# pythoncrazy/jimm

Hardware: NVIDIA H100
Metric: images/sec (higher is better)
Workload: dtype f16

## Files before the change

### include/jimm_b200.h

```cpp
#ifndef JIMM_B200_H_
#define JIMM_B200_H_

#include <stddef.h>
#include <stdint.h>

#if defined(__GNUC__)
#define JIMM_API __attribute__((visibility("default")))
#else
#define JIMM_API
#endif

#ifdef __cplusplus
extern "C" {
#endif

typedef struct jimm_model jimm_model_t;

enum jimm_status { JIMM_OK = 0, JIMM_EINVAL = -1, JIMM_ECUDA = -2, JIMM_EDRIVER = -3, JIMM_ESTATE = -4, JIMM_ENOMEM = -5 };
enum jimm_dtype { JIMM_F32 = 0, JIMM_F16 = 1, JIMM_BF16 = 2, JIMM_I32 = 3 };
enum jimm_kind {
  JIMM_VIT = 0, JIMM_CLIP = 1, JIMM_SIGLIP = 2, JIMM_TOWER = 3 ,
  JIMM_ENCODER = 4 ,
  JIMM_MAPHEAD = 5
};
// ... 70 lines not shown
JIMM_API int jimm_k_layernorm_ex(const float* x, int ldx, int group, int row_off, const int32_t* row_index, const float* scale, const float* bias,
                                 float eps, void* out, int out_type, int ldy, int rows, int D, int reverse, void* stream);
JIMM_API int jimm_k_attention_ex(const void* qkv, int io_type, void* out, int out_type, int B, int S, int H, int causal, int reverse,
                                 void* stream);
JIMM_API int jimm_k_map_attention(const float* q, const void* kv, int io_type, void* out, int out_type, int B, int S, int H, void* stream);
JIMM_API int jimm_k_attention_hd(const void* qkv, int io_type, void* out, int out_type, int B, int S, int H, int head_dim, int causal,
                                 int reverse, void* stream);
JIMM_API int jimm_k_map_attention_hd(const float* q, const void* kv, int io_type, void* out, int out_type, int B, int S, int H, int head_dim,
                                     void* stream);
JIMM_API int jimm_k_patchify(const void* img, int in_type, int B, int H, int W, int C, int P, void* out, int out_type, void* stream);
JIMM_API int jimm_k_patchify_ex(const void* img, int in_type, int B, int H, int W, int C, int P, void* out, int out_type, int rows_per_sample,
                                int ldk, void* stream);
JIMM_API int jimm_k_activation(const float* x, float* y, long long n, int act, void* stream);
JIMM_API int jimm_k_embed(const int32_t* ids, const float* table, const float* pos, float* x, int B, int T, int D, int vocab, void* stream);
JIMM_API int jimm_k_l2_normalize(const float* x, float* out, int ldo, int B, int E, void* stream);
JIMM_API int jimm_k_logits(const float* img, const float* txt, const float* logit_scale, const float* logit_bias, float* logits, int Bi, int Bt,
                  int E, int ldl, void* stream);
typedef struct jimm_preproc_config {
  int height, width;
  int shortest_edge;
  int crop_h, crop_w;
  int resample;
  double rescale_factor;
  float mean[3], std[3];
} jimm_preproc_config_t;
JIMM_API int jimm_preproc_create(const jimm_preproc_config_t* cfg, int device, jimm_preproc_t** out);
JIMM_API int jimm_preproc_output_size(const jimm_preproc_t* p, int H, int W, int* out_h, int* out_w);
JIMM_API int jimm_preproc_run(jimm_preproc_t* p, const uint8_t* img, int B, int H, int W, void* out, int out_dtype, void* stream);
JIMM_API int jimm_preproc_destroy(jimm_preproc_t* p);
JIMM_API int jimm_k_resample_coeffs(int in_size, int out_size, int resample, int* ksize, int* first, int* count, int* kk, int kk_capacity);
JIMM_API int jimm_postprocess(const float* logits, int rows, int cols, int ld, int mode, float* probs, int ldp, int32_t* order, int32_t* argmax,
                              void* stream);
JIMM_API int jimm_k_l2_probe(const void* buf, int rows, int mode, int cluster, int iters, float* ms, void* stream);
JIMM_API int jimm_profile_begin(jimm_model_t* m);
JIMM_API int jimm_profile_end(jimm_model_t* m, double* gemm_ms, double* gemm_flops, long long* gemm_launches);
JIMM_API long long jimm_launch_count(void);
JIMM_API long long jimm_graph_replay_count(void);

#ifdef __cplusplus
}
#endif
#endif
```

### jimm_b200/_lib.py

```python

from __future__ import annotations

import ctypes as C
import os

_HERE = os.path.dirname(os.path.abspath(__file__))
LIB_PATH = os.path.join(_HERE, "libjimm_b200.so")

F32, F16, BF16, I32 = 0, 1, 2, 3
PARAM_TRANSPOSED = 1
KIND_VIT, KIND_CLIP, KIND_SIGLIP, KIND_TOWER, KIND_ENCODER, KIND_MAPHEAD = 0, 1, 2, 3, 4, 5
POOL_CLS, POOL_MAP = 0, 1
ACT_GELU_TANH, ACT_QUICK_GELU = 0, 1
TPOOL_EOT_ARGMAX, TPOOL_LAST = 0, 1


class Config(C.Structure):

    _fields_ = [
        ("kind", C.c_int),
        ("img_size", C.c_int), ("patch", C.c_int), ("in_ch", C.c_int), ("v_width", C.c_int), ("v_layers", C.c_int),
        ("v_heads", C.c_int), ("v_mlp", C.c_int),
        ("pooling", C.c_int),
        ("pre_norm", C.c_int), ("patch_bias", C.c_int), ("v_act", C.c_int),
# ... 35 lines not shown
    "jimm_contrastive_logits": (_i, [_vp, _fp, _i, _fp, _i, _fp, _vp]),
    "jimm_dual_encode": (_i, [_vp, _vp, _i, _i, _ip, _i, _i, _fp, _fp, _vp]),
    "jimm_dual_forward": (_i, [_vp, _vp, _i, _i, _ip, _i, _i, _fp, _vp]),
    "jimm_encoder_forward": (_i, [_vp, _fp, _i, _i, _fp, _vp]),
    "jimm_map_head_forward": (_i, [_vp, _fp, _i, _i, _fp, _vp]),
    "jimm_vit_forward_host": (_i, [_vp, _vp, _i, _i, _fp, _vp]),
    "jimm_dual_forward_host": (_i, [_vp, _vp, _i, _i, _ip, _i, _i, _fp, _vp]),
    "jimm_vit_forward_host_u8": (_i, [_vp, _vp, _vp, _i, _i, _i, _fp, _vp]),
    "jimm_comm_init": (_i, [_vp, _i, _i, _i, C.c_char_p]),
    "jimm_comm_connect": (_i, [_vp, C.c_char_p]),
    "jimm_comm_contrastive_logits": (_i, [_vp, _fp, _fp, _i, _fp, _vp]),
    "jimm_comm_status": (_i, [_vp]),
    "jimm_comm_gathered": (_i, [_vp, C.POINTER(_vp), C.POINTER(_i)]),
    "jimm_profile_begin": (_i, [_vp]),
    "jimm_profile_end": (_i, [_vp, C.POINTER(C.c_double), C.POINTER(C.c_double), C.POINTER(C.c_longlong)]),
    "jimm_k_gemm": (_i, [_i, _i, _vp, _i, _vp, _i, _i, _i, _i, _fp, _i, _fp, _fp, _i, _vp, _i, _i, _i, _i, _i, _i, _vp]),
    "jimm_k_gemm_residual_ln": (_i, [_i, _vp, _i, _vp, _i, _i, _i, _i, _fp, _fp, _i, _fp, _fp, _f, _vp, _i, _i, _ip, _vp]),
    "jimm_k_gemm_ex": (_i, [_i, _i, _vp, _i, _vp, _i, _i, _i, _i, _fp, _i, _fp, _fp, _i, _vp, _i, _i, _i, _i, _i, _i,
                            _i, _i, _i, _i, _i, _fp, _fp, _f, _vp, _i, _i, _ip, _vp]),
    "jimm_k_layernorm": (_i, [_fp, _i, _i, _i, _ip, _fp, _fp, _f, _vp, _i, _i, _i, _i, _vp]),
    "jimm_k_attention": (_i, [_vp, _i, _vp, _i, _i, _i, _i, _i, _vp]),
    "jimm_k_layernorm_ex": (_i, [_fp, _i, _i, _i, _ip, _fp, _fp, _f, _vp, _i, _i, _i, _i, _i, _vp]),
    "jimm_k_attention_ex": (_i, [_vp, _i, _vp, _i, _i, _i, _i, _i, _i, _vp]),
    "jimm_k_map_attention": (_i, [_fp, _vp, _i, _vp, _i, _i, _i, _i, _vp]),
    "jimm_k_attention_hd": (_i, [_vp, _i, _vp, _i, _i, _i, _i, _i, _i, _i, _vp]),
    "jimm_k_map_attention_hd": (_i, [_fp, _vp, _i, _vp, _i, _i, _i, _i, _i, _vp]),
    "jimm_k_patchify": (_i, [_vp, _i, _i, _i, _i, _i, _i, _vp, _i, _vp]),
    "jimm_k_patchify_ex": (_i, [_vp, _i, _i, _i, _i, _i, _i, _vp, _i, _i, _i, _vp]),
    "jimm_k_activation": (_i, [_fp, _fp, C.c_longlong, _i, _vp]),
    "jimm_k_embed": (_i, [_ip, _fp, _fp, _fp, _i, _i, _i, _i, _vp]),
    "jimm_k_l2_normalize": (_i, [_fp, _fp, _i, _i, _i, _vp]),
    "jimm_k_logits": (_i, [_fp, _fp, _fp, _fp, _fp, _i, _i, _i, _i, _vp]),
    "jimm_k_l2_probe": (_i, [_vp, _i, _i, _i, _i, C.POINTER(C.c_float), _vp]),
    "jimm_postprocess": (_i, [_fp, _i, _i, _i, _i, _fp, _i, _ip, _ip, _vp]),
    "jimm_preproc_create": (_i, [C.POINTER(PreprocConfig), _i, C.POINTER(_vp)]),
    "jimm_preproc_output_size": (_i, [_vp, _i, _i, C.POINTER(_i), C.POINTER(_i)]),
    "jimm_preproc_run": (_i, [_vp, _vp, _i, _i, _i, _vp, _i, _vp]),
    "jimm_preproc_destroy": (_i, [_vp]),
    "jimm_k_resample_coeffs": (_i, [_i, _i, _i, C.POINTER(_i), _ip, _ip, _ip, _i]),
}

_lib = None


class JimmError(RuntimeError):
    pass


def load():
    global _lib
    if _lib is not None:
        return _lib
    if not os.path.exists(LIB_PATH):
        raise JimmError(f"{LIB_PATH} not found: build it with `python -m jimm_b200.build` (there is no CPU fallback)")
    lib = C.CDLL(LIB_PATH)
    for name, (res, args) in SIGNATURES.items():
        fn = getattr(lib, name)
        fn.restype = res
        fn.argtypes = args
    _lib = lib
    return lib


def last_error() -> str:
    return load().jimm_last_error().decode("utf-8", "replace")

# ... 9 lines not shown
```

### jimm_b200/csrc/common.cuh

```cuda
#pragma once

#include <cuda.h>
#include <cuda_bf16.h>
#include <cuda_fp16.h>
#include <cuda_runtime.h>
#include <stdint.h>

namespace jimm {

void set_last_error(const char* fmt, ...);

#define JIMM_CUDA_CHECK(expr)                                                                   \
  do {                                                                                          \
    cudaError_t _e = (expr);                                                                    \
    if (_e != cudaSuccess) {                                                                    \
      ::jimm::set_last_error("%s:%d: %s -> %s", __FILE__, __LINE__, #expr, cudaGetErrorString(_e)); \
      return -2;                                                                                \
    }                                                                                           \
  } while (0)

void note_launch();
#define JIMM_LAUNCH_CHECK()                  \
  do {                                       \
    JIMM_CUDA_CHECK(cudaGetLastError());     \
// ... 83 lines not shown
  asm volatile(
      "{\n\t.reg .pred P1;\n\t"
      "WAIT_LOOP:\n\t"
      "mbarrier.try_wait.parity.shared::cta.b64 P1, [%0], %1;\n\t"
      "@P1 bra DONE;\n\t"
      "bra WAIT_LOOP;\n\t"
      "DONE:\n\t}" ::"r"(smem_u32(bar)),
      "r"(parity)
      : "memory");
}

__device__ __forceinline__ bool mbar_test_wait(uint64_t* bar, uint32_t parity) {
  uint32_t ok;
  asm volatile(
      "{\n\t.reg .pred P1;\n\t"
      "mbarrier.test_wait.parity.shared::cta.b64 P1, [%1], %2;\n\t"
      "selp.u32 %0, 1, 0, P1;\n\t}"
      : "=r"(ok)
      : "r"(smem_u32(bar)), "r"(parity)
      : "memory");
  return ok != 0;
}

__device__ __forceinline__ void tma_prefetch_desc(const CUtensorMap* m) {
  asm volatile("prefetch.tensormap [%0];" ::"l"(reinterpret_cast<uint64_t>(m)) : "memory");
}
__device__ __forceinline__ void tma_load_2d(void* smem_dst, const CUtensorMap* m, uint64_t* bar, int c0, int c1) {
  asm volatile(
      "cp.async.bulk.tensor.2d.shared::cluster.global.mbarrier::complete_tx::bytes [%0], [%1, {%3, %4}], [%2];" ::"r"(
          smem_u32(smem_dst)),
      "l"(reinterpret_cast<uint64_t>(m)), "r"(smem_u32(bar)), "r"(c0), "r"(c1)
      : "memory");
}

__device__ __forceinline__ void tma_store_2d(const CUtensorMap* m, uint32_t smem_src, int c0, int c1) {
  asm volatile("cp.async.bulk.tensor.2d.global.shared::cta.bulk_group [%0, {%2, %3}], [%1];" ::"l"(reinterpret_cast<uint64_t>(m)),
               "r"(smem_src), "r"(c0), "r"(c1)
               : "memory");
}
__device__ __forceinline__ void tma_reduce_add_2d(const CUtensorMap* m, uint32_t smem_src, int c0, int c1) {
  asm volatile("cp.reduce.async.bulk.tensor.2d.global.shared::cta.add.tile.bulk_group [%0, {%2, %3}], [%1];" ::"l"(
                   reinterpret_cast<uint64_t>(m)),
               "r"(smem_src), "r"(c0), "r"(c1)
               : "memory");
}
__device__ __forceinline__ void tma_store_3d(const CUtensorMap* m, uint32_t smem_src, int c0, int c1, int c2) {
  asm volatile("cp.async.bulk.tensor.3d.global.shared::cta.bulk_group [%0, {%2, %3, %4}], [%1];" ::"l"(reinterpret_cast<uint64_t>(m)),
               "r"(smem_src), "r"(c0), "r"(c1), "r"(c2)
               : "memory");
}
__device__ __forceinline__ void tma_reduce_add_3d(const CUtensorMap* m, uint32_t smem_src, int c0, int c1, int c2) {
  asm volatile("cp.reduce.async.bulk.tensor.3d.global.shared::cta.add.tile.bulk_group [%0, {%2, %3, %4}], [%1];" ::"l"(
                   reinterpret_cast<uint64_t>(m)),
               "r"(smem_src), "r"(c0), "r"(c1), "r"(c2)
               : "memory");
}
__device__ __forceinline__ void tma_store_commit() { asm volatile("cp.async.bulk.commit_group;" ::: "memory"); }
__device__ __forceinline__ void tma_store_wait_read() { asm volatile("cp.async.bulk.wait_group.read 0;" ::: "memory"); }
__device__ __forceinline__ void tma_store_wait_read1() { asm volatile("cp.async.bulk.wait_group.read 1;" ::: "memory"); }
__device__ __forceinline__ void tma_store_wait_all() { asm volatile("cp.async.bulk.wait_group 0;" ::: "memory"); }

__device__ __forceinline__ uint32_t cluster_ctarank() {
  uint32_t r;
  asm volatile("mov.u32 %0, %%cluster_ctarank;" : "=r"(r));
  return r;
}
__device__ __forceinline__ void cluster_sync_all() {
  asm volatile("barrier.cluster.arrive.release.aligned;\n\tbarrier.cluster.wait.acquire.aligned;" ::: "memory");
}
__device__ __forceinline__ uint32_t mapa_shared(uint32_t local_smem_addr, uint32_t rank) {
  uint32_t r;
  asm volatile("mapa.shared::cluster.u32 %0, %1, %2;" : "=r"(r) : "r"(local_smem_addr), "r"(rank));
  return r;
}
__device__ __forceinline__ void mbar_arrive_cluster(uint32_t cluster_addr) {
  asm volatile("mbarrier.arrive.release.cluster.shared::cluster.b64 _, [%0];" ::"r"(cluster_addr) : "memory");
}
__device__ __forceinline__ uint64_t make_wgmma_desc_sw128(uint32_t smem_addr) {
  uint64_t d = 0;
  d |= static_cast<uint64_t>((smem_addr & 0x3FFFFu) >> 4);
  d |= static_cast<uint64_t>(1) << 16;
  d |= static_cast<uint64_t>(1024 >> 4) << 32;
  d |= static_cast<uint64_t>(1) << 62;
  return d;
}
template <int SW>
__device__ __forceinline__ uint64_t make_wgmma_desc(uint32_t smem_addr, uint32_t lbo) {
  static_assert(SW == 128 || SW == 64 || SW == 32, "swizzle width");
  constexpr uint64_t layout = SW == 128 ? 1 : SW == 64 ? 2 : 3;
  uint64_t d = 0;
  d |= static_cast<uint64_t>((smem_addr & 0x3FFFFu) >> 4);
  d |= static_cast<uint64_t>((lbo >> 4) & 0x3FFFu) << 16;
  d |= static_cast<uint64_t>(8 * SW >> 4) << 32;
  d |= layout << 62;
  return d;
}
__device__ __forceinline__ void wgmma_fence() { asm volatile("wgmma.fence.sync.aligned;" ::: "memory"); }
__device__ __forceinline__ void wgmma_commit() { asm volatile("wgmma.commit_group.sync.aligned;" ::: "memory"); }
template <int N>
__device__ __forceinline__ void wgmma_wait() { asm volatile("wgmma.wait_group.sync.aligned %0;" ::"n"(N) : "memory"); }
template <int R>
__device__ __forceinline__ void wgmma_fence_operands(float (&d)[R]) {
#pragma unroll
  for (int i = 0; i < R; ++i) asm volatile("" : "+f"(d[i])::"memory");
}

#define JIMM_WGMMA_D128                                                                                                                    \
  "{%0, %1, %2, %3, %4, %5, %6, %7, %8, %9, %10, %11, %12, %13, %14, %15, %16, %17, %18, %19, %20, %21, %22, %23, %24, %25, %26, %27, "     \
  "%28, %29, %30, %31, %32, %33, %34, %35, %36, %37, %38, %39, %40, %41, %42, %43, %44, %45, %46, %47, %48, %49, %50, %51, %52, %53, %54, " \
// ... 252 lines not shown
```

### jimm_b200/csrc/gemm.cu

```cuda
#include "gemm.cuh"

#include <stdarg.h>
#include <stdio.h>
#include <stdlib.h>
#include <string.h>

#include <type_traits>

#include "common.cuh"

namespace jimm {

static constexpr int BM = GEMM_TILE_M;
static constexpr int BN = GEMM_TILE_N;
static_assert(BM == 128 && BN == 256, "the warp roles and the wgmma shape below are written for 128 x 256 tiles");
static constexpr int STAGES = 4;
static constexpr int A_STAGE_BYTES = BM * 128;
static constexpr int B_STAGE_BYTES = BN * 128;
static constexpr int STAGE_BYTES = A_STAGE_BYTES + B_STAGE_BYTES;
static constexpr int EPI_WARPS = 8;
static constexpr int EPI_BOX_ROWS = 16;
static constexpr int EPI_BUF_BYTES = EPI_BOX_ROWS * 128;
static constexpr int EPI_BUFS = 2;
static constexpr int EPI_STAGE_BYTES = EPI_WARPS * EPI_BUFS * EPI_BUF_BYTES;
static constexpr int NUM_THREADS = 384;
static constexpr int KERNEL_REGS = 168;

enum OutKind : int { OUT_GENERIC = 0, OUT_H16 = 1, OUT_BF16 = 2, OUT_TF32 = 3, OUT_F32_ADD = 4, OUT_F32 = 5 };

struct EpiDev {
  const float* bias;
  const float* rowadd;
  const float* residual;
  void* out;
  int act, ldr, out_type, ldo, rows_in, rows_out, row_off, mode;
  int M, N;
  int reverse;
  int tok_pad, tok_off;
  const float* ln_scale;
  const float* ln_bias;
  void* ln_out;
  int* ln_cnt;
  int ln_out_type, ln_ldo;
  float ln_eps;
};

template <int ACT>
__device__ __forceinline__ float act_ct(float v) {
// ... 252 lines not shown
          if (epi.residual) v += epi.residual[static_cast<size_t>(out_row) * epi.ldr + col];
          store1(epi, out_row, col, v);
        }
      }
    }
  }
}

template <typename T, int OUT, int ACT>
__global__ void __launch_bounds__(NUM_THREADS, 1)
gemm_wgmma_kernel(const __grid_constant__ CUtensorMap map_a, const __grid_constant__ CUtensorMap map_b,
                  const __grid_constant__ CUtensorMap map_c, const EpiDev epi, int K) {
  constexpr int BK = 128 / sizeof(T);
  constexpr int UK = 32 / sizeof(T);
  constexpr bool FUSE_LN = OUT == OUT_F32_ADD && ACT == ACT_FUSE_LN;
  constexpr int EPI_ACT = ACT == ACT_FUSE_LN ? static_cast<int>(ACT_NONE) : ACT;
  constexpr int PRODUCER_REGS = FUSE_LN ? 152 : 40;
  constexpr int CONSUMER_REGS = FUSE_LN ? 176 : 232;
  static_assert(128 * PRODUCER_REGS + 256 * CONSUMER_REGS <= NUM_THREADS * KERNEL_REGS, "register split exceeds the CTA's allocation");

  extern __shared__ uint8_t smem_raw[];
  uint8_t* smem = reinterpret_cast<uint8_t*>((reinterpret_cast<uintptr_t>(smem_raw) + 1023) & ~static_cast<uintptr_t>(1023));
  uint8_t* smem_a = smem;
  uint8_t* smem_b = smem + STAGES * A_STAGE_BYTES;
  uint8_t* epi_stage = smem + STAGES * STAGE_BYTES;
  LnQueue* lnq = reinterpret_cast<LnQueue*>(epi_stage + EPI_STAGE_BYTES);
  uint64_t* full_bar = reinterpret_cast<uint64_t*>(lnq + 1);
  uint64_t* empty_bar = full_bar + STAGES;

  const int warp_idx = threadIdx.x >> 5;
  const int lane = threadIdx.x & 31;
  const int M = epi.M, N = epi.N;
  const int m_tiles = (M + BM - 1) / BM, n_tiles = (N + BN - 1) / BN;
  const int num_tiles = m_tiles * n_tiles;
  const int num_kb = (K + BK - 1) / BK;

  pdl_launch_dependents();
  if (warp_idx == 0 && lane == 0) {
    tma_prefetch_desc(&map_a);
    tma_prefetch_desc(&map_b);
    if constexpr (OUT != OUT_GENERIC) tma_prefetch_desc(&map_c);
    for (int s = 0; s < STAGES; ++s) {
      mbar_init(&full_bar[s], 1);
      mbar_init(&empty_bar[s], EPI_WARPS);
    }
    fence_barrier_init();
  }
  if constexpr (FUSE_LN) {
    if (warp_idx == 1) {
      for (int i = lane; i < LNQ; i += 32) lnq->slot[i] = -1;
      if (lane == 0) lnq->head = lnq->tail = lnq->done = 0;
    }
  }
  __syncthreads();
  pdl_wait();

  if (warp_idx < 4) {
    setmaxnreg<KERNEL_REGS, PRODUCER_REGS>();
    if (warp_idx == 0) {
      if (lane == 0) {
        int stage = 0;
        uint32_t phase = 0;
        for (int tile = blockIdx.x; tile < num_tiles; tile += gridDim.x) {
          const int tv = epi.reverse ? num_tiles - 1 - tile : tile;
          const int m_blk = tv / n_tiles, n_blk = tv - m_blk * n_tiles;
          for (int kb = 0; kb < num_kb; ++kb) {
            mbar_wait(&empty_bar[stage], phase ^ 1);
            mbar_arrive_expect_tx(&full_bar[stage], STAGE_BYTES);
            tma_load_2d(smem_a + stage * A_STAGE_BYTES, &map_a, &full_bar[stage], kb * BK, m_blk * BM);
            tma_load_2d(smem_b + stage * B_STAGE_BYTES, &map_b, &full_bar[stage], kb * BK, n_blk * BN);
            if (++stage == STAGES) { stage = 0; phase ^= 1; }
          }
        }
      }
    } else if constexpr (FUSE_LN) {
      ln_worker<T>(epi, lnq, lane);
    }
  } else {
    setmaxnreg<KERNEL_REGS, CONSUMER_REGS>();
    const int wg = (warp_idx - 4) >> 2;
    const int wq = warp_idx & 3;
    uint8_t* tbuf0 = epi_stage + (warp_idx - 4) * EPI_BUFS * EPI_BUF_BYTES;
    int stage = 0;
    uint32_t phase = 0, box_count = 0;
    int ln_rg = -1, ln_cols = 0;
    float acc[128];
    for (int tile = blockIdx.x; tile < num_tiles; tile += gridDim.x) {
      const int tv = epi.reverse ? num_tiles - 1 - tile : tile;
      const int m_blk = tv / n_tiles, n_blk = tv - m_blk * n_tiles;
      int prev = -1;
      for (int kb = 0; kb < num_kb; ++kb) {
        mbar_wait(&full_bar[stage], phase);
        const uint64_t adesc = make_wgmma_desc_sw128(smem_u32(smem_a + stage * A_STAGE_BYTES + wg * 64 * 128));
        const uint64_t bdesc = make_wgmma_desc_sw128(smem_u32(smem_b + stage * B_STAGE_BYTES));
        wgmma_fence_operands(acc);
        wgmma_fence();
#pragma unroll
        for (int k = 0; k < BK / UK; ++k)
          wgmma_m64n256_ss<Traits<T>::KIND>(acc, adesc + static_cast<uint64_t>(2 * k), bdesc + static_cast<uint64_t>(2 * k), (kb | k) != 0 ? 1u : 0u);
        wgmma_commit();
        wgmma_fence_operands(acc);
        if (prev >= 0) {
          wgmma_wait<1>();
          if (lane == 0) mbar_arrive(&empty_bar[prev]);
        }
        prev = stage;
        if (++stage == STAGES) { stage = 0; phase ^= 1; }
      }
      wgmma_wait<0>();
      wgmma_fence_operands(acc);
      if (lane == 0) mbar_arrive(&empty_bar[prev]);

      const int row_base = m_blk * BM + wg * 64 + wq * 16;
      const int n_tile0 = n_blk * BN;
      if constexpr (OUT == OUT_GENERIC) {
        epilogue_generic(epi, acc, lane, row_base, n_tile0);
      } else {
        if (row_base < M) epilogue_tma<OUT, EPI_ACT>(&map_c, epi, acc, tbuf0, lane, row_base, n_tile0, box_count);
        if constexpr (FUSE_LN) {
          if (lane == 0 && ln_rg >= 0) ln_publish(epi, lnq, ln_rg, ln_cols);
          ln_rg = (row_base & ~31) < M ? row_base >> 5 : -1;
          ln_cols = min(BN, N - n_tile0);
        }
      }
    }
    if constexpr (FUSE_LN) {
      if (lane == 0) {
        if (ln_rg >= 0) ln_publish(epi, lnq, ln_rg, ln_cols);
        __threadfence_block();
        atomicAdd(&lnq->done, 1);
      }
    }
    if constexpr (OUT != OUT_GENERIC) {
      if (lane == 0) tma_store_wait_all();
    }
  }
}

template <typename T>
__global__ void gemm_simt_kernel(const T* __restrict__ A, int lda, const T* __restrict__ B, int ldb, int K, EpiDev epi) {
  __shared__ float As[16][17], Bs[16][17];
  const int tx = threadIdx.x, ty = threadIdx.y;
  const int row = blockIdx.y * 16 + ty, col = blockIdx.x * 16 + tx;
  float acc = 0.f;
  for (int k0 = 0; k0 < K; k0 += 16) {
    const int ar = blockIdx.y * 16 + ty, ak = k0 + tx;
    As[ty][tx] = (ar < epi.M && ak < K) ? to_float(A[static_cast<size_t>(ar) * lda + ak]) : 0.f;
    const int br = blockIdx.x * 16 + ty, bk = k0 + tx;
    Bs[ty][tx] = (br < epi.N && bk < K) ? to_float(B[static_cast<size_t>(br) * ldb + bk]) : 0.f;
    __syncthreads();
#pragma unroll
    for (int k = 0; k < 16; ++k) acc += As[ty][k] * Bs[tx][k];
    __syncthreads();
  }
  if (row < epi.M && col < epi.N) {
    int out_row, add_row;
    remap_row(epi, row, out_row, add_row);
    float v = acc;
    if (epi.bias) v += epi.bias[col];
    v = apply_act(v, epi.act);
    if (epi.rowadd) v += epi.rowadd[static_cast<size_t>(add_row) * epi.N + col];
    if (epi.residual) v += epi.residual[static_cast<size_t>(out_row) * epi.ldr + col];
    store1(epi, out_row, col, v);
  }
}

static constexpr int SMEM_BYTES = STAGES * STAGE_BYTES + EPI_STAGE_BYTES + static_cast<int>(sizeof(LnQueue)) + 2 * STAGES * 8 + 1024;
static_assert(SMEM_BYTES <= 232448, "exceeds 227 KB of shared memory");
typedef CUresult (*PFN_encodeTiled)(CUtensorMap*, CUtensorMapDataType, cuuint32_t, void*, const cuuint64_t*, const cuuint64_t*,
// ... 43 lines not shown
  const size_t es = dtype_size(dtype);
  CUtensorMapDataType dt = (dtype == DT_F32 || dtype == DT_TF32) ? CU_TENSOR_MAP_DATA_TYPE_FLOAT32
                                           : (dtype == DT_F16 ? CU_TENSOR_MAP_DATA_TYPE_FLOAT16 : CU_TENSOR_MAP_DATA_TYPE_BFLOAT16);
  cuuint64_t dims[3] = {static_cast<cuuint64_t>(N), static_cast<cuuint64_t>(S), static_cast<cuuint64_t>(B)};
  cuuint64_t strides[2] = {static_cast<cuuint64_t>(ld) * es, static_cast<cuuint64_t>(S) * ld * es};
  cuuint32_t box[3] = {static_cast<cuuint32_t>(128 / es), EPI_BOX_ROWS, 1};
  cuuint32_t estr[3] = {1, 1, 1};
  CUresult r = enc(map, dt, 3, const_cast<void*>(ptr), dims, strides, box, estr, CU_TENSOR_MAP_INTERLEAVE_NONE,
                   CU_TENSOR_MAP_SWIZZLE_128B, CU_TENSOR_MAP_L2_PROMOTION_L2_256B, CU_TENSOR_MAP_FLOAT_OOB_FILL_NONE);
  if (r != CUDA_SUCCESS) { set_last_error("cuTensorMapEncodeTiled(3d) failed: CUresult %d", static_cast<int>(r)); return -3; }
  return 0;
}
static int make_map_3d_f32(CUtensorMap* map, const void* ptr, int B, int S, int N, int ld) { return make_tensor_map_3d(map, DT_F32, ptr, B, S, N, ld); }

int make_tensor_map_2d(CUtensorMap* map, int dtype, const void* ptr, int rows, int cols, int ld, int box_rows) {
  return make_map(map, dtype, ptr, rows, cols, ld, box_rows);
}

int device_sm_count() {
  static int sms[DeviceOnce::kMaxDevices] = {};
  int dev = 0;
  cudaGetDevice(&dev);
  if (dev < 0 || dev >= DeviceOnce::kMaxDevices) dev = 0;
  if (sms[dev] == 0) {
    int n = 0;
    cudaDeviceGetAttribute(&n, cudaDevAttrMultiProcessorCount, dev);
    const char* env = getenv("JIMM_NUM_SMS");
    if (env && atoi(env) > 0) n = atoi(env);
    sms[dev] = n;
  }
  return sms[dev];
}

static int check_epi(const GemmEpilogue& e, int N) {
  if (e.out == nullptr) { set_last_error("gemm: null output"); return -1; }
  if (e.ldo < N) { set_last_error("gemm: ldo (%d) < N (%d)", e.ldo, N); return -1; }
  return 0;
}
int gemm_plan_init(GemmPlan* plan, int dtype, const void* A, int lda, const void* B, int ldb, int M, int N, int K,
                   const GemmEpilogue& epi) {
  if (M <= 0 || N <= 0 || K <= 0) { set_last_error("gemm: bad shape %dx%dx%d", M, N, K); return -1; }
  if (int rc = check_epi(epi, N)) return rc;
  if (epi.tok_pad != 0) {
    if (epi.tok_pad < 0 || epi.tok_pad % EPI_BOX_ROWS != 0 || M % epi.tok_pad != 0 || epi.tok_off < 0 || epi.tok_S <= 0) {
      set_last_error("gemm: token scatter needs tok_pad a positive multiple of %d dividing M (tok_pad=%d M=%d tok_off=%d tok_S=%d)", EPI_BOX_ROWS,
                     epi.tok_pad, M, epi.tok_off, epi.tok_S);
      return -1;
    }
    if (epi.residual != epi.out || epi.ldr != epi.ldo || epi.out_type != DT_F32) {
      set_last_error("gemm: token scatter reduce-adds into an fp32 output that is also the residual");
      return -1;
    }
  }
  if (int rc = make_map(&plan->map_a, dtype, A, M, K, lda, BM)) return rc;
  if (int rc = make_map(&plan->map_b, dtype, B, N, K, ldb, BN)) return rc;
  plan->M = M; plan->N = N; plan->K = K; plan->dtype = dtype; plan->epi = epi;
  memset(&plan->map_c, 0, sizeof(plan->map_c));
  if (plan->epi.mode == 2) {
    const size_t es = dtype_size(epi.out_type);
    const bool ok = epi.rowadd == nullptr && epi.rows_in == 0 && (static_cast<size_t>(N) * es) % 16 == 0 &&
                    (epi.residual == nullptr || (epi.residual == epi.out && epi.ldr == epi.ldo && epi.out_type == DT_F32)) &&
                    (static_cast<size_t>(epi.ldo) * es) % 16 == 0 && (reinterpret_cast<uintptr_t>(epi.out) & 15) == 0 &&
                    (epi.bias == nullptr || ((reinterpret_cast<uintptr_t>(epi.bias) & 15) == 0 && N % 4 == 0)) &&
                    !(epi.residual && epi.act != ACT_NONE);
    if (ok && epi.tok_pad > 0) {
      if (int rc = make_map_3d_f32(&plan->map_c, epi.out, M / epi.tok_pad, epi.tok_S, N, epi.ldo)) return rc;
    } else if (ok) {
      if (int rc = make_map(&plan->map_c, epi.out_type, epi.out, M, N, epi.ldo, EPI_BOX_ROWS)) return rc;
    } else {
      plan->epi.mode = 0;
    }
  }
  if (epi.tok_pad > 0 && plan->epi.mode != 2) {
    set_last_error("gemm: the token scatter needs the TMA epilogue (mode 2, no activation, 16-byte aligned output / bias, N %% 4 == 0)");
    return -1;
  }
  return 0;
}

static EpiDev to_dev(const GemmEpilogue& e, int M, int N) {
  EpiDev d;
  d.bias = e.bias; d.rowadd = e.rowadd; d.residual = e.residual; d.out = e.out;
  d.act = e.act; d.ldr = e.ldr; d.out_type = e.out_type; d.ldo = e.ldo;
  d.rows_in = e.rows_in; d.rows_out = e.rows_out; d.row_off = e.row_off; d.mode = e.mode;
  d.M = M; d.N = N;
  d.tok_pad = e.tok_pad; d.tok_off = e.tok_off;
  d.reverse = e.reverse;
  d.ln_scale = e.ln_scale; d.ln_bias = e.ln_bias; d.ln_out = e.ln_out; d.ln_cnt = e.ln_cnt;
  d.ln_out_type = e.ln_out_type; d.ln_ldo = e.ln_ldo; d.ln_eps = e.ln_eps;
  return d;
}

template <typename T, int OUT, int ACT>
static int launch_one(const GemmPlan* p, int M, cudaStream_t stream) {
  static DeviceOnce attr_set;
  if (attr_set.first()) {
    JIMM_CUDA_CHECK(cudaFuncSetAttribute(gemm_wgmma_kernel<T, OUT, ACT>, cudaFuncAttributeMaxDynamicSharedMemorySize, SMEM_BYTES));
    cudaFuncAttributes fa;
    JIMM_CUDA_CHECK(cudaFuncGetAttributes(&fa, gemm_wgmma_kernel<T, OUT, ACT>));
    if (fa.numRegs != KERNEL_REGS) {
      set_last_error("gemm: kernel compiled with %d registers per thread, the warpgroup register split assumes %d", fa.numRegs, KERNEL_REGS);
      return -2;
    }
  }
  const int tiles = ((M + BM - 1) / BM) * ((p->N + BN - 1) / BN);
  const int grid = tiles < device_sm_count() ? tiles : device_sm_count();
  JIMM_CUDA_CHECK(launch_k(gemm_wgmma_kernel<T, OUT, ACT>, dim3(grid), dim3(NUM_THREADS), SMEM_BYTES, stream, 1, true, p->map_a, p->map_b,
                           p->map_c, to_dev(p->epi, M, p->N), p->K));
  note_launch();
  return 0;
}

template <typename T, int OUT>
static int launch_act(const GemmPlan* p, int M, cudaStream_t stream) {
  switch (p->epi.act) {
    case ACT_GELU_TANH: return launch_one<T, OUT, ACT_GELU_TANH>(p, M, stream);
    case ACT_QUICK_GELU: return launch_one<T, OUT, ACT_QUICK_GELU>(p, M, stream);
    default: return launch_one<T, OUT, ACT_NONE>(p, M, stream);
  }
}

template <typename T>
static int launch_tc(const GemmPlan* p, int M, cudaStream_t stream) {
  const GemmEpilogue& e = p->epi;
  if (e.mode != 2) return launch_one<T, OUT_GENERIC, ACT_NONE>(p, M, stream);
  if (e.residual) return gemm_fuses_ln(p, M) ? launch_one<T, OUT_F32_ADD, ACT_FUSE_LN>(p, M, stream) : launch_one<T, OUT_F32_ADD, ACT_NONE>(p, M, stream);
  switch (e.out_type) {
    case DT_F16: return launch_act<T, OUT_H16>(p, M, stream);
    case DT_BF16: return launch_act<T, OUT_BF16>(p, M, stream);
    case DT_TF32: return launch_act<T, OUT_TF32>(p, M, stream);
    default: return launch_act<T, OUT_F32>(p, M, stream);
  }
}

int gemm_fuses_ln(const GemmPlan* p, int ) {
  const int nv = p->N >> 7;
  const bool width_ok = p->N % 128 == 0 && (nv <= 4 || nv == 6 || nv == 8 || nv == 9);
  const int want = p->dtype == DT_F16 ? DT_F16 : p->dtype == DT_BF16 ? DT_BF16 : DT_TF32;
  return p->epi.ln_cnt != nullptr && p->epi.ln_out_type == want && width_ok && p->epi.mode == 2 && p->epi.residual != nullptr && p->epi.tok_pad == 0;
}

// ... 33 lines not shown
```

### jimm_b200/csrc/gemm.cuh

```cuda
#pragma once
#include <cuda.h>
#include <cuda_runtime.h>
#include <stdint.h>

namespace jimm {

enum DType : int { DT_F32 = 0, DT_F16 = 1, DT_BF16 = 2, DT_TF32 = 3 };
enum Act : int { ACT_NONE = 0, ACT_GELU_TANH = 1, ACT_QUICK_GELU = 2 };

inline size_t dtype_size(int dt) { return (dt == DT_F32 || dt == DT_TF32) ? 4 : 2; }

constexpr int GEMM_TILE_M = 128;
constexpr int GEMM_TILE_N = 256;

struct GemmEpilogue {
  const float* bias = nullptr;
  int act = ACT_NONE;
  const float* rowadd = nullptr;
  const float* residual = nullptr;
  int ldr = 0;
  void* out = nullptr;
  int out_type = DT_F32;
  int ldo = 0;
  int tok_pad = 0, tok_off = 0, tok_S = 0;
  int reverse = 0;
  int rows_in = 0, rows_out = 0, row_off = 0;
  int mode = 2;
  const float* ln_scale = nullptr;
  const float* ln_bias = nullptr;
  void* ln_out = nullptr;
  int ln_out_type = DT_F16, ln_ldo = 0;
  float ln_eps = 1e-6f;
  int* ln_cnt = nullptr;
};

struct GemmPlan {
  CUtensorMap map_a, map_b, map_c;
  int M = 0, N = 0, K = 0;
  int dtype = DT_F16;
  GemmEpilogue epi;
};

int gemm_plan_init(GemmPlan* plan, int dtype, const void* A, int lda, const void* B, int ldb, int M, int N, int K,
                   const GemmEpilogue& epi);
int gemm_plan_run(const GemmPlan* plan, int M_override, cudaStream_t stream, int reverse = 0);

int gemm_simt_run(int dtype, const void* A, int lda, const void* B, int ldb, int M, int N, int K, const GemmEpilogue& epi,
                  cudaStream_t stream);

int gemm_fuses_ln(const GemmPlan* plan, int M_override);

int device_sm_count();

}
```

### jimm_b200/csrc/model.cu

```cuda
#include <stdarg.h>
#include <stdio.h>
#include <stdlib.h>
#include <string.h>

#include <atomic>
#include <cmath>
#include <map>
#include <tuple>
#include <memory>
#include <string>
#include <vector>

#include "../../include/jimm_b200.h"
#include "comm.cuh"
#include "common.cuh"
#include "gemm.cuh"
#include "kernels.cuh"

namespace jimm {

static thread_local char g_err[1024] = "";
void set_last_error(const char* fmt, ...) {
  va_list ap;
  va_start(ap, fmt);
// ... 1084 lines not shown

static int ensure_copy_stream(jimm_model* m) {
  if (m->copy_stream) return 0;
  JIMM_CUDA_CHECK(cudaStreamCreateWithFlags(&m->copy_stream, cudaStreamNonBlocking));
  for (int i = 0; i < jimm_model::kHostSlices; ++i) {
    JIMM_CUDA_CHECK(cudaEventCreateWithFlags(&m->ev_copied[i], cudaEventDisableTiming));
    JIMM_CUDA_CHECK(cudaEventCreateWithFlags(&m->ev_consumed[i], cudaEventDisableTiming));
  }
  JIMM_CUDA_CHECK(cudaEventCreateWithFlags(&m->ev_start, cudaEventDisableTiming));
  return 0;
}

static void host_slices(const jimm_model* m, int nb, int* sizes, size_t bytes_per_image = 0) {
  for (int i = 0; i < jimm_model::kHostSlices; ++i) sizes[i] = 0;
  sizes[0] = nb;
  if (const char* env = getenv("JIMM_HOST_SLICES")) {
    int k = 0, acc = 0;
    for (const char* q = env; *q && k < jimm_model::kHostSlices - 1;) {
      const int v = atoi(q);
      if (v <= 0 || acc + v >= nb) break;
      sizes[k++] = v;
      acc += v;
      while (*q && *q != ',') ++q;
      if (*q == ',') ++q;
    }
    sizes[k] = nb - acc;
    return;
  }
  if (nb < 128) return;
  if (bytes_per_image && static_cast<size_t>(nb) * bytes_per_image < (static_cast<size_t>(64) << 20)) return;
  static int head_div = -1;
  if (head_div < 0) { const char* env = getenv("JIMM_HOST_HEAD_DIV"); head_div = (env && atoi(env) > 0) ? atoi(env) : 4; }
  const int S = m->vis.S, D = m->vis.D, Mm = m->vis.enc.c.M;
  const int sms = device_sm_count();
  auto cost = [&](int n) {
    const long mt = (static_cast<long>(n) * S + GEMM_TILE_M - 1) / GEMM_TILE_M;
    auto rounds = [&](int N) { return (mt * ((N + GEMM_TILE_N - 1) / GEMM_TILE_N) + sms - 1) / sms; };
    return static_cast<double>(D) * rounds(3 * D) + static_cast<double>(D) * rounds(D) + static_cast<double>(D) * rounds(Mm) +
           static_cast<double>(Mm) * rounds(D);
  };
  int best = nb / head_div;
  double best_cost = 1e30;
  for (int c0 = nb / head_div; c0 <= nb / 3; ++c0) {
    const double cst = cost(c0) + cost(nb - c0) + 1e-3 * c0 * D;
    if (cst < best_cost) { best_cost = cst; best = c0; }
  }
  sizes[0] = best;
  sizes[1] = nb - best;
}

static int vit_forward_host_impl(jimm_model_t* m, const void* img_host, int in_dtype, int B, float* out_host, cudaStream_t s,
                                 jimm_preproc_t* pre, int Hin, int Win) {
  JIMM_TRY(ensure_copy_stream(m));
  const size_t img_elems = static_cast<size_t>(m->vis.img) * m->vis.img * m->vis.C;
  const size_t src_bytes = pre ? static_cast<size_t>(Hin) * Win * 3 : img_elems * dtype_size(in_dtype);
  const int tower_dtype = pre ? (m->cdt == DT_TF32 ? JIMM_F32 : m->cdt) : in_dtype;
  const int od = vision_out_dim(m);
  const int kind = pre ? 1 : 0;
  if (pre) {
    const size_t need = static_cast<size_t>(m->max_batch) * src_bytes;
    if (need > m->ws.in_u8_bytes) {
      JIMM_CUDA_CHECK(cudaDeviceSynchronize());
      if (m->ws.in_u8) cudaFree(m->ws.in_u8);
      m->ws.in_u8 = nullptr; m->ws.in_u8_bytes = 0;
      JIMM_CUDA_CHECK(cudaMalloc(&m->ws.in_u8, need));
      m->ws.in_u8_bytes = need;
      m->host_chain = false;
    }
  }
  for (int b0 = 0; b0 < B; b0 += m->max_batch) {
// ... 178 lines not shown
    e.ln_scale = ln_scale; e.ln_bias = ln_bias; e.ln_out = ln_out; e.ln_out_type = ln_out_type == JIMM_F32 ? DT_TF32 : ln_out_type; e.ln_ldo = ln_ldo;
    e.ln_eps = ln_eps; e.ln_cnt = ln_counters;
  }
  cudaStream_t s = static_cast<cudaStream_t>(stream);
  if (impl == 1) {
    if (plan_M != M || reverse || tok_pad || ln_counters) {
      set_last_error("jimm_k_gemm_ex: the SIMT GEMM has no plan rows, reverse walk, token scatter or fused LayerNorm");
      return JIMM_EINVAL;
    }
    return gemm_simt_run(dtype, A, lda, B, ldb, M, N, K, e, s);
  }
  GemmPlan p;
  JIMM_TRY(gemm_plan_init(&p, dtype, A, lda, B, ldb, plan_M, N, K, e));
  if (ln_counters && !gemm_fuses_ln(&p, M)) {
    set_last_error("gemm: this shape does not take the fused LayerNorm path (needs N = 128 x {1,2,3,4,6,8,9}, aligned operands, "
                   "LayerNorm output in the operand type)");
    return JIMM_EINVAL;
  }
  return gemm_plan_run(&p, M, s, reverse);
}
int jimm_k_gemm(int impl, int dtype, const void* A, int lda, const void* B, int ldb, int M, int N, int K, const float* bias, int act,
                const float* rowadd, const float* residual, int ldr, void* out, int out_type, int ldo, int rows_in, int rows_out,
                int row_off, int epi_mode, void* stream) {
  return jimm_k_gemm_ex(impl, dtype, A, lda, B, ldb, M, N, K, bias, act, rowadd, residual, ldr, out, out_type, ldo, rows_in, rows_out, row_off,
                        epi_mode, M, 0, 0, 0, 0, nullptr, nullptr, 0.f, nullptr, 0, 0, nullptr, stream);
}
int jimm_k_gemm_residual_ln(int dtype, const void* A, int lda, const void* B, int ldb, int M, int N, int K, const float* bias, float* x, int ldx,
                            const float* ln_scale, const float* ln_bias, float eps, void* ln_out, int ln_out_type, int ln_ldo, int* counters,
                            void* stream) {
  if (!counters) { set_last_error("jimm_k_gemm_residual_ln: null counters"); return JIMM_EINVAL; }
  return jimm_k_gemm_ex(0, dtype, A, lda, B, ldb, M, N, K, bias, 0, nullptr, x, ldx, x, JIMM_F32, ldx, 0, 0, 0, 2, M, 0, 0, 0, 0, ln_scale,
                        ln_bias, eps, ln_out, ln_out_type, ln_ldo, counters, stream);
}
int jimm_k_layernorm_ex(const float* x, int ldx, int group, int row_off, const int32_t* row_index, const float* scale, const float* bias,
                        float eps, void* out, int out_type, int ldy, int rows, int D, int reverse, void* stream) {
  return layernorm_run(x, ldx, group, row_off, row_index, scale, bias, eps, out, out_type, ldy, rows, D, static_cast<cudaStream_t>(stream), reverse);
}
int jimm_k_layernorm(const float* x, int ldx, int group, int row_off, const int32_t* row_index, const float* scale, const float* bias,
                     float eps, void* out, int out_type, int ldy, int rows, int D, void* stream) {
  return jimm_k_layernorm_ex(x, ldx, group, row_off, row_index, scale, bias, eps, out, out_type, ldy, rows, D, 0, stream);
}
int jimm_k_attention_hd(const void* qkv, int io_type, void* out, int out_type, int B, int S, int H, int head_dim, int causal, int reverse,
                        void* stream) {
  return attention_run(qkv, io_type, out, out_type, B, S, H, head_dim, causal, static_cast<cudaStream_t>(stream), reverse);
}
int jimm_k_attention_ex(const void* qkv, int io_type, void* out, int out_type, int B, int S, int H, int causal, int reverse, void* stream) {
  return jimm_k_attention_hd(qkv, io_type, out, out_type, B, S, H, 64, causal, reverse, stream);
}
int jimm_k_attention(const void* qkv, int io_type, void* out, int out_type, int B, int S, int H, int causal, void* stream) {
  return jimm_k_attention_ex(qkv, io_type, out, out_type, B, S, H, causal, 0, stream);
}
int jimm_k_map_attention_hd(const float* q, const void* kv, int io_type, void* out, int out_type, int B, int S, int H, int head_dim, void* stream) {
  return map_attention_run(q, kv, io_type, out, out_type, B, S, H, head_dim, static_cast<cudaStream_t>(stream));
}
int jimm_k_map_attention(const float* q, const void* kv, int io_type, void* out, int out_type, int B, int S, int H, void* stream) {
  return jimm_k_map_attention_hd(q, kv, io_type, out, out_type, B, S, H, 64, stream);
}
int jimm_k_patchify_ex(const void* img, int in_type, int B, int H, int W, int C, int P, void* out, int out_type, int rows_per_sample, int ldk,
                       void* stream) {
  return patchify_run(img, in_type, B, H, W, C, P, out, out_type, static_cast<cudaStream_t>(stream), rows_per_sample, ldk);
}
int jimm_k_patchify(const void* img, int in_type, int B, int H, int W, int C, int P, void* out, int out_type, void* stream) {
  return jimm_k_patchify_ex(img, in_type, B, H, W, C, P, out, out_type, 0, 0, stream);
}
int jimm_k_activation(const float* x, float* y, long long n, int act, void* stream) {
  if (n < 0 || (n > 0 && (!x || !y))) { set_last_error("jimm_k_activation: bad arguments"); return JIMM_EINVAL; }
// ... 15 lines not shown
```

### jimm_b200/csrc/probe.cu

```cuda
#include "../../include/jimm_b200.h"
#include "common.cuh"
#include "gemm.cuh"

namespace jimm {

int make_tensor_map_2d(CUtensorMap* map, int dtype, const void* ptr, int rows, int cols, int ld, int box_rows);

namespace {

constexpr int PB_STAGES = 12;
constexpr int PB_STAGE_BYTES = 128 * 128;

__device__ __forceinline__ void tma_load_2d_multicast(void* smem_dst, const CUtensorMap* m, uint64_t* bar, int c0, int c1, uint16_t mask) {
  asm volatile(
      "cp.async.bulk.tensor.2d.shared::cluster.global.mbarrier::complete_tx::bytes.multicast::cluster [%0], [%1, {%3, %4}], [%2], %5;" ::"r"(
          smem_u32(smem_dst)),
      "l"(reinterpret_cast<uint64_t>(m)), "r"(smem_u32(bar)), "r"(c0), "r"(c1), "h"(mask)
      : "memory");
}

template <int CS>
__global__ void __launch_bounds__(64, 1) l2_probe_kernel(const __grid_constant__ CUtensorMap map_full, const __grid_constant__ CUtensorMap map_part,
                                                         int mode, int iters, int total_rows) {
  extern __shared__ uint8_t smem_raw[];
  uint8_t* smem = reinterpret_cast<uint8_t*>((reinterpret_cast<uintptr_t>(smem_raw) + 1023) & ~static_cast<uintptr_t>(1023));
  uint64_t* full = reinterpret_cast<uint64_t*>(smem + PB_STAGES * PB_STAGE_BYTES);
  uint64_t* empty = full + PB_STAGES;
  const uint32_t rank = CS > 1 ? cluster_ctarank() : 0;
  const int cluster_id = blockIdx.x / CS;
  const bool shared_writes = CS > 1 && mode == 2;
  if (threadIdx.x == 0) {
    for (int i = 0; i < PB_STAGES; ++i) {
      mbar_init(&full[i], 1);
      mbar_init(&empty[i], shared_writes ? CS : 1);
    }
    fence_barrier_init();
  }
  __syncthreads();
  if (CS > 1) cluster_sync_all();
  const int tiles = total_rows / 128;
  if (threadIdx.x == 0) {
    int st = 0;
    uint32_t ph = 0;
    for (int it = 0; it < iters; ++it) {
      const long long tile = mode == 0 ? (static_cast<long long>(blockIdx.x) * iters + it) : (static_cast<long long>(cluster_id) * iters + it);
      const int row = static_cast<int>((tile * 7919) % tiles) * 128;
      mbar_wait(&empty[st], ph ^ 1);
      mbar_arrive_expect_tx(&full[st], PB_STAGE_BYTES);
      if (mode == 2 && CS > 1) {
        constexpr int part = 128 / CS;
        tma_load_2d_multicast(smem + st * PB_STAGE_BYTES + rank * part * 128, &map_part, &full[st], 0, row + rank * part,
                              static_cast<uint16_t>((1u << CS) - 1));
// ... 68 lines not shown
```

Before: 11950.

## Run GEMM in 2-CTA clusters with TMA multicast of the B tile

The persistent WGMMA GEMM now launches as 2-CTA clusters along M. Each CTA loads its own A tile and half of the shared B tile, multicasting that half to both CTAs. Stage release becomes cross-CTA, with each consumer arriving on both CTAs' empty barriers. This halves B traffic from L2, but adds cluster synchronization and ties the two CTAs' progress together. The host-side cost model and grid size now count clusters, using an occupancy query, instead of SMs.

```diff
diff --git a/include/jimm_b200.h b/include/jimm_b200.h
--- a/include/jimm_b200.h
+++ b/include/jimm_b200.h
@@ -126,6 +126,7 @@
 JIMM_API int jimm_postprocess(const float* logits, int rows, int cols, int ld, int mode, float* probs, int ldp, int32_t* order, int32_t* argmax,
                               void* stream);
 JIMM_API int jimm_k_l2_probe(const void* buf, int rows, int mode, int cluster, int iters, float* ms, void* stream);
+JIMM_API int jimm_gemm_max_clusters(void);
 JIMM_API int jimm_profile_begin(jimm_model_t* m);
 JIMM_API int jimm_profile_end(jimm_model_t* m, double* gemm_ms, double* gemm_flops, long long* gemm_launches);
 JIMM_API long long jimm_launch_count(void);
diff --git a/jimm_b200/_lib.py b/jimm_b200/_lib.py
--- a/jimm_b200/_lib.py
+++ b/jimm_b200/_lib.py
@@ -91,6 +91,7 @@
     "jimm_k_l2_normalize": (_i, [_fp, _fp, _i, _i, _i, _vp]),
     "jimm_k_logits": (_i, [_fp, _fp, _fp, _fp, _fp, _i, _i, _i, _i, _vp]),
     "jimm_k_l2_probe": (_i, [_vp, _i, _i, _i, _i, C.POINTER(C.c_float), _vp]),
+    "jimm_gemm_max_clusters": (_i, []),
     "jimm_postprocess": (_i, [_fp, _i, _i, _i, _i, _fp, _i, _ip, _ip, _vp]),
     "jimm_preproc_create": (_i, [C.POINTER(PreprocConfig), _i, C.POINTER(_vp)]),
     "jimm_preproc_output_size": (_i, [_vp, _i, _i, C.POINTER(_i), C.POINTER(_i)]),
diff --git a/jimm_b200/csrc/common.cuh b/jimm_b200/csrc/common.cuh
--- a/jimm_b200/csrc/common.cuh
+++ b/jimm_b200/csrc/common.cuh
@@ -139,6 +139,13 @@
       "l"(reinterpret_cast<uint64_t>(m)), "r"(smem_u32(bar)), "r"(c0), "r"(c1)
       : "memory");
 }
+__device__ __forceinline__ void tma_load_2d_multicast(void* smem_dst, const CUtensorMap* m, uint64_t* bar, int c0, int c1, uint16_t mask) {
+  asm volatile(
+      "cp.async.bulk.tensor.2d.shared::cluster.global.mbarrier::complete_tx::bytes.multicast::cluster [%0], [%1, {%3, %4}], [%2], %5;" ::"r"(
+          smem_u32(smem_dst)),
+      "l"(reinterpret_cast<uint64_t>(m)), "r"(smem_u32(bar)), "r"(c0), "r"(c1), "h"(mask)
+      : "memory");
+}
 
 __device__ __forceinline__ void tma_store_2d(const CUtensorMap* m, uint32_t smem_src, int c0, int c1) {
   asm volatile("cp.async.bulk.tensor.2d.global.shared::cta.bulk_group [%0, {%2, %3}], [%1];" ::"l"(reinterpret_cast<uint64_t>(m)),
@@ -182,6 +189,9 @@
 }
 __device__ __forceinline__ void mbar_arrive_cluster(uint32_t cluster_addr) {
   asm volatile("mbarrier.arrive.release.cluster.shared::cluster.b64 _, [%0];" ::"r"(cluster_addr) : "memory");
+}
+__device__ __forceinline__ void mbar_arrive_remote(uint32_t cluster_addr) {
+  asm volatile("mbarrier.arrive.shared::cluster.b64 _, [%0];" ::"r"(cluster_addr) : "memory");
 }
 __device__ __forceinline__ uint64_t make_wgmma_desc_sw128(uint32_t smem_addr) {
   uint64_t d = 0;
diff --git a/jimm_b200/csrc/gemm.cu b/jimm_b200/csrc/gemm.cu
--- a/jimm_b200/csrc/gemm.cu
+++ b/jimm_b200/csrc/gemm.cu
@@ -13,7 +13,11 @@
 
 static constexpr int BM = GEMM_TILE_M;
 static constexpr int BN = GEMM_TILE_N;
+static constexpr int CM = GEMM_CLUSTER_M;
 static_assert(BM == 128 && BN == 256, "the warp roles and the wgmma shape below are written for 128 x 256 tiles");
+static_assert(CM == 2, "the B multicast and the two-CTA stage release below are written for 2-CTA clusters");
+static constexpr int B_PART_ROWS = BN / CM;
+static_assert(B_PART_ROWS % 8 == 0, "a B part must start on a swizzle-atom boundary");
 static constexpr int STAGES = 4;
 static constexpr int A_STAGE_BYTES = BM * 128;
 static constexpr int B_STAGE_BYTES = BN * 128;
@@ -332,8 +336,10 @@
   const int lane = threadIdx.x & 31;
   const int M = epi.M, N = epi.N;
   const int m_tiles = (M + BM - 1) / BM, n_tiles = (N + BN - 1) / BN;
-  const int num_tiles = m_tiles * n_tiles;
+  const int num_groups = (m_tiles + CM - 1) / CM * n_tiles;
   const int num_kb = (K + BK - 1) / BK;
+  const int rank = static_cast<int>(cluster_ctarank());
+  const int cluster_id = blockIdx.x / CM, num_clusters = gridDim.x / CM;
 
   pdl_launch_dependents();
   if (warp_idx == 0 && lane == 0) {
@@ -342,7 +348,7 @@
     if constexpr (OUT != OUT_GENERIC) tma_prefetch_desc(&map_c);
     for (int s = 0; s < STAGES; ++s) {
       mbar_init(&full_bar[s], 1);
-      mbar_init(&empty_bar[s], EPI_WARPS);
+      mbar_init(&empty_bar[s], CM * EPI_WARPS);
     }
     fence_barrier_init();
   }
@@ -352,7 +358,7 @@
       if (lane == 0) lnq->head = lnq->tail = lnq->done = 0;
     }
   }
-  __syncthreads();
+  cluster_sync_all();
   pdl_wait();
 
   if (warp_idx < 4) {
@@ -361,14 +367,16 @@
       if (lane == 0) {
         int stage = 0;
         uint32_t phase = 0;
-        for (int tile = blockIdx.x; tile < num_tiles; tile += gridDim.x) {
-          const int tv = epi.reverse ? num_tiles - 1 - tile : tile;
-          const int m_blk = tv / n_tiles, n_blk = tv - m_blk * n_tiles;
+        for (int grp = cluster_id; grp < num_groups; grp += num_clusters) {
+          const int gv = epi.reverse ? num_groups - 1 - grp : grp;
+          const int m_grp = gv / n_tiles, n_blk = gv - m_grp * n_tiles;
+          const int m_blk = m_grp * CM + rank;
           for (int kb = 0; kb < num_kb; ++kb) {
             mbar_wait(&empty_bar[stage], phase ^ 1);
             mbar_arrive_expect_tx(&full_bar[stage], STAGE_BYTES);
             tma_load_2d(smem_a + stage * A_STAGE_BYTES, &map_a, &full_bar[stage], kb * BK, m_blk * BM);
-            tma_load_2d(smem_b + stage * B_STAGE_BYTES, &map_b, &full_bar[stage], kb * BK, n_blk * BN);
+            tma_load_2d_multicast(smem_b + stage * B_STAGE_BYTES + rank * B_PART_ROWS * 128, &map_b, &full_bar[stage], kb * BK,
+                                  n_blk * BN + rank * B_PART_ROWS, static_cast<uint16_t>((1u << CM) - 1));
             if (++stage == STAGES) { stage = 0; phase ^= 1; }
           }
         }
@@ -385,9 +393,14 @@
     uint32_t phase = 0, box_count = 0;
     int ln_rg = -1, ln_cols = 0;
     float acc[128];
-    for (int tile = blockIdx.x; tile < num_tiles; tile += gridDim.x) {
-      const int tv = epi.reverse ? num_tiles - 1 - tile : tile;
-      const int m_blk = tv / n_tiles, n_blk = tv - m_blk * n_tiles;
+    auto release = [&](int s) {
+      mbar_arrive(&empty_bar[s]);
+      mbar_arrive_remote(mapa_shared(smem_u32(&empty_bar[s]), static_cast<uint32_t>(rank ^ 1)));
+    };
+    for (int grp = cluster_id; grp < num_groups; grp += num_clusters) {
+      const int gv = epi.reverse ? num_groups - 1 - grp : grp;
+      const int m_grp = gv / n_tiles, n_blk = gv - m_grp * n_tiles;
+      const int m_blk = m_grp * CM + rank;
       int prev = -1;
       for (int kb = 0; kb < num_kb; ++kb) {
         mbar_wait(&full_bar[stage], phase);
@@ -402,14 +415,14 @@
         wgmma_fence_operands(acc);
         if (prev >= 0) {
           wgmma_wait<1>();
-          if (lane == 0) mbar_arrive(&empty_bar[prev]);
+          if (lane == 0) release(prev);
         }
         prev = stage;
         if (++stage == STAGES) { stage = 0; phase ^= 1; }
       }
       wgmma_wait<0>();
       wgmma_fence_operands(acc);
-      if (lane == 0) mbar_arrive(&empty_bar[prev]);
+      if (lane == 0) release(prev);
 
       const int row_base = m_blk * BM + wg * 64 + wq * 16;
       const int n_tile0 = n_blk * BN;
@@ -435,6 +448,8 @@
       if (lane == 0) tma_store_wait_all();
     }
   }
+  __syncwarp();
+  cluster_sync_all();
 }
 
 template <typename T>
@@ -544,6 +559,38 @@
   return sms[dev];
 }
 
+int gemm_max_clusters() {
+  static int clusters[DeviceOnce::kMaxDevices] = {};
+  int dev = 0;
+  cudaGetDevice(&dev);
+  if (dev < 0 || dev >= DeviceOnce::kMaxDevices) dev = 0;
+  if (clusters[dev] == 0) {
+    auto kernel = gemm_wgmma_kernel<__half, OUT_H16, ACT_NONE>;
+    cudaError_t e = cudaFuncSetAttribute(kernel, cudaFuncAttributeMaxDynamicSharedMemorySize, SMEM_BYTES);
+    cudaLaunchConfig_t cfg = {};
+    cfg.gridDim = dim3(CM);
+    cfg.blockDim = dim3(NUM_THREADS);
+    cfg.dynamicSmemBytes = SMEM_BYTES;
+    cudaLaunchAttribute attr;
+    attr.id = cudaLaunchAttributeClusterDimension;
+    attr.val.clusterDim.x = CM;
+    attr.val.clusterDim.y = 1;
+    attr.val.clusterDim.z = 1;
+    cfg.attrs = &attr;
+    cfg.numAttrs = 1;
+    int n = 0;
+    if (e == cudaSuccess) e = cudaOccupancyMaxActiveClusters(&n, kernel, &cfg);
+    if (e != cudaSuccess || n <= 0) {
+      set_last_error("gemm: no %d-CTA cluster of the GEMM kernel (%d threads, %d B of shared memory per CTA) fits on device %d: %s", CM,
+                     NUM_THREADS, SMEM_BYTES, dev, e != cudaSuccess ? cudaGetErrorString(e) : "occupancy query returned 0 clusters");
+      return 0;
+    }
+    const int cap = device_sm_count() / CM;
+    clusters[dev] = n < cap ? n : (cap > 0 ? cap : 1);
+  }
+  return clusters[dev];
+}
+
 static int check_epi(const GemmEpilogue& e, int N) {
   if (e.out == nullptr) { set_last_error("gemm: null output"); return -1; }
   if (e.ldo < N) { set_last_error("gemm: ldo (%d) < N (%d)", e.ldo, N); return -1; }
@@ -565,7 +612,7 @@
     }
   }
   if (int rc = make_map(&plan->map_a, dtype, A, M, K, lda, BM)) return rc;
-  if (int rc = make_map(&plan->map_b, dtype, B, N, K, ldb, BN)) return rc;
+  if (int rc = make_map(&plan->map_b, dtype, B, N, K, ldb, B_PART_ROWS)) return rc;
   plan->M = M; plan->N = N; plan->K = K; plan->dtype = dtype; plan->epi = epi;
   memset(&plan->map_c, 0, sizeof(plan->map_c));
   if (plan->epi.mode == 2) {
@@ -615,10 +662,12 @@
       return -2;
     }
   }
-  const int tiles = ((M + BM - 1) / BM) * ((p->N + BN - 1) / BN);
-  const int grid = tiles < device_sm_count() ? tiles : device_sm_count();
-  JIMM_CUDA_CHECK(launch_k(gemm_wgmma_kernel<T, OUT, ACT>, dim3(grid), dim3(NUM_THREADS), SMEM_BYTES, stream, 1, true, p->map_a, p->map_b,
-                           p->map_c, to_dev(p->epi, M, p->N), p->K));
+  const int groups = ((M + BM - 1) / BM + CM - 1) / CM * ((p->N + BN - 1) / BN);
+  const int max_clusters = gemm_max_clusters();
+  if (max_clusters <= 0) return -2;
+  const int clusters = groups < max_clusters ? groups : max_clusters;
+  JIMM_CUDA_CHECK(launch_k(gemm_wgmma_kernel<T, OUT, ACT>, dim3(CM * clusters), dim3(NUM_THREADS), SMEM_BYTES, stream, CM, true, p->map_a,
+                           p->map_b, p->map_c, to_dev(p->epi, M, p->N), p->K));
   note_launch();
   return 0;
 }
diff --git a/jimm_b200/csrc/gemm.cuh b/jimm_b200/csrc/gemm.cuh
--- a/jimm_b200/csrc/gemm.cuh
+++ b/jimm_b200/csrc/gemm.cuh
@@ -12,6 +12,7 @@
 
 constexpr int GEMM_TILE_M = 128;
 constexpr int GEMM_TILE_N = 256;
+constexpr int GEMM_CLUSTER_M = 2;
 
 struct GemmEpilogue {
   const float* bias = nullptr;
@@ -51,5 +52,6 @@
 int gemm_fuses_ln(const GemmPlan* plan, int M_override);
 
 int device_sm_count();
+int gemm_max_clusters();
 
 }
diff --git a/jimm_b200/csrc/model.cu b/jimm_b200/csrc/model.cu
--- a/jimm_b200/csrc/model.cu
+++ b/jimm_b200/csrc/model.cu
@@ -1140,10 +1140,11 @@
   static int head_div = -1;
   if (head_div < 0) { const char* env = getenv("JIMM_HOST_HEAD_DIV"); head_div = (env && atoi(env) > 0) ? atoi(env) : 4; }
   const int S = m->vis.S, D = m->vis.D, Mm = m->vis.enc.c.M;
-  const int sms = device_sm_count();
+  const int clusters = gemm_max_clusters() > 0 ? gemm_max_clusters() : 1;
   auto cost = [&](int n) {
     const long mt = (static_cast<long>(n) * S + GEMM_TILE_M - 1) / GEMM_TILE_M;
-    auto rounds = [&](int N) { return (mt * ((N + GEMM_TILE_N - 1) / GEMM_TILE_N) + sms - 1) / sms; };
+    const long mg = (mt + GEMM_CLUSTER_M - 1) / GEMM_CLUSTER_M;
+    auto rounds = [&](int N) { return (mg * ((N + GEMM_TILE_N - 1) / GEMM_TILE_N) + clusters - 1) / clusters; };
     return static_cast<double>(D) * rounds(3 * D) + static_cast<double>(D) * rounds(D) + static_cast<double>(D) * rounds(Mm) +
            static_cast<double>(Mm) * rounds(D);
   };
@@ -1388,6 +1389,7 @@
   return jimm_k_gemm_ex(0, dtype, A, lda, B, ldb, M, N, K, bias, 0, nullptr, x, ldx, x, JIMM_F32, ldx, 0, 0, 0, 2, M, 0, 0, 0, 0, ln_scale,
                         ln_bias, eps, ln_out, ln_out_type, ln_ldo, counters, stream);
 }
+int jimm_gemm_max_clusters(void) { return gemm_max_clusters(); }
 int jimm_k_layernorm_ex(const float* x, int ldx, int group, int row_off, const int32_t* row_index, const float* scale, const float* bias,
                         float eps, void* out, int out_type, int ldy, int rows, int D, int reverse, void* stream) {
   return layernorm_run(x, ldx, group, row_off, row_index, scale, bias, eps, out, out_type, ldy, rows, D, static_cast<cudaStream_t>(stream), reverse);
diff --git a/jimm_b200/csrc/probe.cu b/jimm_b200/csrc/probe.cu
--- a/jimm_b200/csrc/probe.cu
+++ b/jimm_b200/csrc/probe.cu
@@ -10,14 +10,6 @@
 
 constexpr int PB_STAGES = 12;
 constexpr int PB_STAGE_BYTES = 128 * 128;
-
-__device__ __forceinline__ void tma_load_2d_multicast(void* smem_dst, const CUtensorMap* m, uint64_t* bar, int c0, int c1, uint16_t mask) {
-  asm volatile(
-      "cp.async.bulk.tensor.2d.shared::cluster.global.mbarrier::complete_tx::bytes.multicast::cluster [%0], [%1, {%3, %4}], [%2], %5;" ::"r"(
-          smem_u32(smem_dst)),
-      "l"(reinterpret_cast<uint64_t>(m)), "r"(smem_u32(bar)), "r"(c0), "r"(c1), "h"(mask)
-      : "memory");
-}
 
 template <int CS>
 __global__ void __launch_bounds__(64, 1) l2_probe_kernel(const __grid_constant__ CUtensorMap map_full, const __grid_constant__ CUtensorMap map_part,
```

Measured after the change: 12120 (median of 6 runs). 1.01x the previous value.
